# mkln/spamtree

Measured on AMD Instinct MI355X. Metric: Gibbs iterations/sec + achieved HBM GB/s, n=1e6 grid, 1/2/4/8 MI355X, higher is better.
Workload: dtype f64

## Files before the change

include/spamtree_hip.h:

```cpp
#ifndef SPAMTREE_HIP_H
#define SPAMTREE_HIP_H

#include <stdint.h>

#ifdef __cplusplus
extern "C" {
#endif

#define ST_OK 0
#define ST_ERR_CHOL_ROOT 1
#define ST_ERR_CHOL_REF 2
#define ST_ERR_CHOL_LEAF 3
#define ST_ERR_CHOL_SAMPLE_REF 10
#define ST_ERR_CHOL_SAMPLE_LEAF 11
#define ST_ERR_USAGE (-1)
#define ST_ERR_HIP (-2)
#define ST_ERR_TOPOLOGY (-3)
#define ST_ERR_UNSUPPORTED (-4)

#define ST_MAX_Q 6
#define ST_MAX_ANCESTORS 24

typedef struct st_handle_s *st_handle;

// ... 68 lines not shown
int st_get_block(st_handle h, int slot, int64_t u, double *negRiH, double *Ri);
int st_get_comps(st_handle h, int slot, double *logdetCi_comps, double *loglik_w_comps);

int st_algorithmic_bytes(st_handle h, double *out5, double *flops3);
int st_probe_peaks(int device, int64_t bytes, int reps, double *out3);
int st_probe_math(int32_t fn, const double *x, int64_t n, int32_t device, double *out);
#define ST_N_KERNEL_FAMILIES 8
int st_profile_enable(st_handle h, int enable);
int st_profile_get(st_handle h, double *ms_total, int64_t *launches);
int st_profile_levels(st_handle h, int32_t *n_levels, double *ms_by_level, double *bytes_by_level, int32_t cap);
#define ST_KERNEL_GENERIC_LDS 0
#define ST_KERNEL_GENERIC_SCRATCH 1
#define ST_KERNEL_MFMA 2
#define ST_KERNEL_QUAD 3
#define ST_KERNEL_BIGMFMA 4
#define ST_KERNEL_WIDE 5
#define ST_KERNEL_LCHAIN 6
#define ST_KERNEL_LCHAIN_REF 7
int st_level_info(st_handle h, int32_t *n_levels, int32_t *kernel, int32_t *max_m, int32_t *max_P, int32_t *n_blocks, int32_t cap);
#define ST_ROUTE_NONE 0
#define ST_ROUTE_A_SLOTS 3
int st_route_info(st_handle h, int32_t *n_levels, int32_t *phase_a, int32_t *phase_b, int32_t *phase_p, int32_t cap);
const char *st_route_name(int32_t code);
int st_synchronize(st_handle h);
void *st_stream(st_handle h);

int st_cross_covariance_ag10(const double *coords1, const int64_t *mv1, int64_t n1, const double *coords2, const int64_t *mv2,
                             int64_t n2, const double *ai1, const double *ai2, const double *phi_i, const double *thetamv,
                             const double *Dmat, int32_t q, int32_t device, double *out);
int st_summary_reset(st_handle h);
int st_summary_accumulate(st_handle h, uint64_t seed, uint32_t iter);
int st_summary_get(st_handle h, double *w_mean, double *yhat_mean, int64_t *n_accumulated);
int st_summary_reserve(st_handle h, int64_t keep);
int st_summary_quantile(st_handle h, double q, double *w_q, double *yhat_q);

int st_points_set(st_handle h, int64_t n_new, const double *coords, const int64_t *mv, const int64_t *anchor, const double *X);
int st_points_predict(st_handle h, int mode, const double *z, uint64_t seed, uint32_t iter, double *w_new, double *cond_mean,
                      double *cond_var, double *yhat_new);
int st_points_info(st_handle h, int32_t *route, int64_t *n_groups, double *alg_bytes, double *flops);
const char *st_points_route_name(int32_t code);

int st_points_accumulate(st_handle h, uint64_t seed, uint32_t iter, double *w_new, double *cond_mean, double *cond_var, double *yhat_new);
int st_points_summary_reset(st_handle h);
int st_points_summary_reserve(st_handle h, int64_t keep);
int st_points_summary_get(st_handle h, double *mean, double *var, double *w_mean, double *yhat_mean, int64_t *n_accumulated);
int st_points_summary_quantile(st_handle h, double q, double *w_q, double *yhat_q);
// ... 29 lines not shown
```

spamtree_amd/_lib.py:

```python
import ctypes as C
import os

HERE = os.path.dirname(os.path.abspath(__file__))
LIB_PATH = os.environ.get("SPAMTREE_LIB") or os.path.join(HERE, "libspamtree_hip.so")

c_dp = C.POINTER(C.c_double)
c_ip = C.POINTER(C.c_int64)


class StProblem(C.Structure):
    _fields_ = [("n_all", C.c_int64), ("d", C.c_int32), ("q", C.c_int32), ("p", C.c_int32), ("n_groups", C.c_int32),
                ("n_blocks", C.c_int64), ("y", c_dp), ("X", c_dp), ("coords", c_dp), ("mv_id", c_ip),
                ("res_is_ref", c_ip), ("block_names", c_ip), ("block_groups", c_ip), ("indexing_ptr", c_ip),
                ("indexing_idx", c_ip), ("parents_ptr", c_ip), ("parents_idx", c_ip), ("children_ptr", c_ip),
                ("children_idx", c_ip)]


class StOptions(C.Structure):
    _fields_ = [("device", C.c_int32), ("reference_quirks", C.c_int32), ("rank", C.c_int32), ("world", C.c_int32),
                ("force_generic", C.c_int32), ("reserved", C.c_int32)]


H = C.c_void_p
SIGNATURES = {
# ... 14 lines not shown
    "st_sample_w_loglik": (C.c_int, [H, c_dp, C.c_uint64, C.c_uint32, C.c_int, c_dp]),
    "st_sample_w_loglik_begin": (C.c_int, [H, c_dp, C.c_uint64, C.c_uint32, C.c_int]),
    "st_sample_w_loglik_end": (C.c_int, [H, c_dp]),
    "st_predict": (C.c_int, [H, C.c_int]),
    "st_beta_stats": (C.c_int, [H, c_dp]),
    "st_tausq_stats": (C.c_int, [H, c_dp, c_ip]),
    "st_xtx": (C.c_int, [H, c_dp]),
    "st_yhat": (C.c_int, [H, c_dp, C.c_uint64, C.c_uint32, c_dp]),
    "st_block_dims": (C.c_int, [H, C.c_int64, c_ip, c_ip, C.POINTER(C.c_int32), C.POINTER(C.c_int32)]),
    "st_get_block": (C.c_int, [H, C.c_int, C.c_int64, c_dp, c_dp]),
    "st_get_comps": (C.c_int, [H, C.c_int, c_dp, c_dp]),
    "st_algorithmic_bytes": (C.c_int, [H, c_dp, c_dp]),
    "st_factor_ahead_enable": (C.c_int, [H, C.c_int]),
    "st_probe_peaks": (C.c_int, [C.c_int, C.c_int64, C.c_int, c_dp]),
    "st_probe_math": (C.c_int, [C.c_int32, c_dp, C.c_int64, C.c_int32, c_dp]),
    "st_profile_enable": (C.c_int, [H, C.c_int]),
    "st_profile_get": (C.c_int, [H, c_dp, c_ip]),
    "st_profile_levels": (C.c_int, [H, C.POINTER(C.c_int32), c_dp, c_dp, C.c_int32]),
    "st_level_info": (C.c_int, [H, C.POINTER(C.c_int32), C.POINTER(C.c_int32), C.POINTER(C.c_int32), C.POINTER(C.c_int32),
                                C.POINTER(C.c_int32), C.c_int32]),
    "st_route_info": (C.c_int, [H, C.POINTER(C.c_int32), C.POINTER(C.c_int32), C.POINTER(C.c_int32), C.POINTER(C.c_int32),
                                C.c_int32]),
    "st_route_name": (C.c_char_p, [C.c_int32]),
    "st_synchronize": (C.c_int, [H]),
    "st_stream": (C.c_void_p, [H]),
    "st_set_stream": (C.c_int, [H, C.c_void_p]),
    "st_shard_plan": (C.c_int, [C.POINTER(StProblem), C.c_int32, c_ip, C.POINTER(C.c_int32)]),
    "st_shard_plan_opt": (C.c_int, [C.POINTER(StProblem), C.POINTER(StOptions), C.c_int32, c_ip, C.POINTER(C.c_int32)]),
    "st_shard_info": (C.c_int, [H, C.POINTER(C.c_int32), C.POINTER(C.c_int32), C.POINTER(C.c_int32), c_ip, c_ip]),
    "st_factor_local": (C.c_int, [H, C.c_int, c_dp, C.c_int]),
    "st_factor_enqueue": (C.c_int, [H, C.c_int, c_dp, C.c_int]),
    "st_factor_finish": (C.c_int, [H, c_dp]),
    "st_factor_is_async": (C.c_int, [H]),
    "st_loglik_local": (C.c_int, [H, C.c_int]),
    "st_mg_pack_comps": (C.c_int, [H, C.c_int, C.POINTER(C.c_void_p), c_ip]),
    "st_mg_finish": (C.c_int, [H, c_dp]),
    "st_sample_w_local": (C.c_int, [H, c_dp, C.c_uint64, C.c_uint32]),
    "st_mg_top_region": (C.c_int, [H, C.POINTER(C.c_void_p), c_ip]),
    "st_sample_w_top": (C.c_int, [H]),
    "st_mg_pack_w": (C.c_int, [H, C.POINTER(C.c_void_p), c_ip]),
    "st_mg_unpack_w": (C.c_int, [H]),
    "st_mg_gather_w_pack": (C.c_int, [H, C.POINTER(C.c_void_p), C.POINTER(C.c_void_p), c_ip]),
    "st_mg_gather_w_unpack": (C.c_int, [H]),
    "st_cross_covariance_ag10": (C.c_int, [c_dp, c_ip, C.c_int64, c_dp, c_ip, C.c_int64, c_dp, c_dp, c_dp, c_dp, c_dp, C.c_int32,
                                           C.c_int32, c_dp]),
    "st_summary_reset": (C.c_int, [H]),
# ... 70 lines not shown
```

spamtree_amd/csrc/factor_quad.hpp:

```cpp
#pragma once

struct Quad {
  int g0, nu;
  int Jc, Pc;
};

struct QuadArgs {
  const Blk *blks;
  const int *anc_idx;
  const Grp *grps;
  const Quad *quads;
  int nquad;
  const double *cx, *cy;
  const int *mv;
  const double *w;
  double *panels;
  double *logdet_c, *loglik_c;
  int *errflag;
  const long long *gdesc;
  int gd_stride;
  int ldS;
  int wave_chol;
  int predict;
  const double *z;
  double *w_out;
  int mode;
  double *vscr;
  int vtiles;
};

enum { QM_FULL = 0, QM_VONLY = 1, QM_TFROMV = 2 };
__host__ __device__ constexpr int quad_vtiles(int nkx) { return 2 + 2 * ((4 * nkx + 31) / 32); }

#define RFL(x) __builtin_amdgcn_readfirstlane(x)

constexpr int QUAD_LEAF_KH = 5;
__host__ __device__ constexpr int quad_lds_stride(int nkx) {
  int s = 4 * nkx + 24 > 186 ? 4 * nkx + 24 : 186;
  while ((s & 1) || ((s >> 1) & 1) == 0) ++s;
  return s;
}

#ifdef ST_DEFS_FACTOR_QUAD
__device__ __forceinline__ void dma_row(const double *src, double *dst, int Kb, int lane, bool two) {
  if (2 * lane < Kb) __builtin_amdgcn_global_load_lds((q_glb_void *)(src + 2 * lane), (q_lds_void *)dst, 16, 0, 0);
  if (two) {
    if (128 + 2 * lane < Kb) __builtin_amdgcn_global_load_lds((q_glb_void *)(src + 128 + 2 * lane), (q_lds_void *)(dst + 128), 16, 0, 0);
  }
}

template <int NU, int NKX, int NKT, bool ISREF, bool WCH = true>
__global__ __launch_bounds__(128 * NU, 2) void k_factor_quad(QuadArgs A, CovPar cp) {
  constexpr int NTQ = 128 * NU, NW = 2 * NU;
  static_assert(NU >= 2, "s_g overlays two rows of s_e2");
// ... 16 lines not shown
  __shared__ double s_sx[PMAX], s_sy[PMAX], s_wpa[PMAX];
  __shared__ int s_smv[PMAX];
  __shared__ double s_exp2[64];
  __shared__ double s_cvr[QMAX * QMAX], s_cva[QMAX * QMAX], s_cva2[QMAX * QMAX], s_cvp[QMAX];
  __shared__ int s_rlen[PMAX];
  __shared__ long long s_rsrc[PMAX];
  double (*s_g)[32] = s_e2;
  double (*s_gp)[32] = s_hv;

  const int tid = threadIdx.x, lane = tid & 63, l15 = lane & 15, l4 = lane >> 4, ttid = tid & 127;
  const int wid = RFL(tid >> 6), u = wid >> 1, jt = (wid & 1) ^ ((wid >> 2) & 1);
  constexpr int ldS = quad_lds_stride(NKX);
  double *arena = lds;
  double *zrow = arena + (size_t)NU * 16 * ldS;
  double *xch = zrow + ldS;

  STAMP_DECL
  int qidx = blockIdx.x;
  {
    const int per = A.nquad >> 3;
    if (qidx < per * 8) qidx = (qidx & 7) * per + (qidx >> 3);
  }
  const Quad Q = A.quads[qidx];
  const int Jc = Q.Jc, Pc = Q.Pc, nu = Q.nu;

  long long *gdl = (long long *)arena;
  const int gds = A.gd_stride;
  for (int e = tid; e < nu * gds; e += NTQ) {
    const int uu = e / gds, i = e - uu * gds;
    gdl[e] = A.gdesc[(size_t)(Q.g0 + uu) * gds + i];
  }
  for (int k = tid; k < ldS; k += NTQ) zrow[k] = 0.0;
  if (tid < 64) s_exp2[tid] = EXP2_64[tid];
  if (cp.q > 1 && tid >= 64 && tid < 64 + QMAX * QMAX) {
    const int e = tid - 64;
    s_cvr[e] = cp.rate[e]; s_cva[e] = cp.amp[e]; s_cva2[e] = cp.amp2[e];
    if (e < QMAX) s_cvp[e] = cp.phi[e];
  }
  __syncthreads();
  if (tid < NU) {
    int M = 0, P = 0, blk0 = 0, nblk = 0, isref = 0, J = 0, pm = 0;
    long long row0 = 0, prow = 0, ppan = 0;
    if (tid < nu) {
      const long long *g = gdl + (size_t)tid * gds;
      row0 = g[0];
      M = (int)(g[2] & 0xffffffffLL); P = (int)(g[2] >> 32);
// ... 85 lines not shown
    for (int rr = 0; rr < RP; ++rr) {
      const int cc = c0 + min(wid + NW * rr, sr - 1);
      lv[rr] = s_rlen[cc]; sv[rr] = s_rsrc[cc];
    }
#pragma unroll
    for (int rr = 0; rr < RP; ++rr) {
      const int row = wid + NW * rr;
      const int len = RFL(lv[rr]);
      rlen_nx[rr] = len;
      if (row < sr) dma_row(A.panels + sv[rr], buf + (size_t)row * ldS, len, lane, len > 128);
    }
  };
  auto priv_rows = [&](int sp) { return sp == 0 ? p_sr0 : (pmu > 16 ? pmu - p_sr0 : 0); };
  auto priv_issue = [&](int sp, int stride) {
    const int r0 = sp == 0 ? 0 : p_sr0, sr = priv_rows(sp);
    const double *src = A.panels + s_ppan[u] + (size_t)r0 * p_Kb;
    double *buf = arena + (size_t)u * stride * ldS;
#pragma unroll
    for (int rr = 0; rr < 8; ++rr) {
      const int row = jt + 2 * rr;
      if (row < sr) dma_row(src + (size_t)row * p_Kb, buf + (size_t)row * ldS, p_Kb, lane, true);
    }
  };
  if constexpr (ISREF) { if (nit > 0) issue(0, arena); }
  else { if (pmmax > 0) priv_issue(0, 16); }

  double kx[NKX];
  if (QM != QM_TFROMV) {
    const int jc = jt * 16 + l15;
    const bool cok = jc < Mu;
    const double mx = s_colx[u][jc], my = s_coly[u][jc];
    const int mvj = s_colmv[u][jc];
    double *kb = (ISREF ? arena + (size_t)32 * ldS : xch) + (size_t)wid * (KH * 64) + lane;
#pragma unroll
    for (int hpass = 0; hpass < NPASS; ++hpass) {
      const int st0 = hpass * KH;
      if (4 * st0 < Pu) {
        if (cp.q == 1) {
          const double s2 = cp.ai1[0], nphi = -cp.tmv[0];
#pragma unroll 1
          for (int i = 0; i < KH; ++i) {
            const int k = 4 * (st0 + i) + l4;
            double ax = s_sx[min(k, PMAX - 1)], ay = s_sy[min(k, PMAX - 1)];
            if constexpr (!ISREF) {
              if (k >= Pc) { ax = s_px[u][(k - Pc) & 31]; ay = s_py[u][(k - Pc) & 31]; }
            }
            const double dx = ax - mx, dy = ay - my;
            const double v = s2 * cov_exp_tab(nphi * cov_sqrt(fma(dx, dx, dy * dy)), s_exp2);
            kb[i * 64] = (cok && k < Pu) ? v : 0.0;
          }
        } else {
          const int qn = cp.q;
#pragma unroll 1
          for (int i = 0; i < KH; ++i) {
            const int k = 4 * (st0 + i) + l4;
            const double *pxs = &s_sx[min(k, PMAX - 1)], *pys = &s_sy[min(k, PMAX - 1)];
            const int *pvs = &s_smv[min(k, PMAX - 1)];
            if constexpr (!ISREF) {
              if (k >= Pc) { pxs = &s_px[u][(k - Pc) & 31]; pys = &s_py[u][(k - Pc) & 31]; pvs = &s_pmv[u][(k - Pc) & 31]; }
            }
            const int av = *pvs;
            const double dx = *pxs - mx, dy = *pys - my;
            const double hd = cov_sqrt(dx * dx + dy * dy);
            const int ij = av * qn + mvj;
            double v = s_cva[ij] * cov_exp_tab(-s_cvr[ij] * hd, s_exp2);
            v = fma(s_cva2[ij], cov_exp_tab(-s_cvp[av] * hd, s_exp2), v);
            kb[i * 64] = (cok && k < Pu) ? v : 0.0;
          }
        }
#pragma unroll
        for (int i = 0; i < KH; ++i)
          if (st0 + i < NKX) kx[st0 + i] = kb[i * 64];
      } else {
#pragma unroll
        for (int i = 0; i < KH; ++i)
          if (st0 + i < NKX) kx[st0 + i] = 0.0;
      }
    }
  }
  STAMP(1);
  d4 tacc[NKT];
#pragma unroll
  for (int n = 0; n < NKT; ++n) tacc[n] = (d4){0.0, 0.0, 0.0, 0.0};
  d4 rown = (d4){0.0, 0.0, 0.0, 0.0}, rcross = rown;
  double dacc = 0.0;
  double hacc = 0.0;
// ... 472 lines not shown
```

spamtree_amd/csrc/spamtree_hip.hip:

```cpp

#include "st_device.hpp"
#include "factor_generic.hpp"
#include "factor_mfma.hpp"
#include "chol_blocked.hpp"
#include "factor_quad.hpp"
#include "factor_big.hpp"
#include "factor_wide.hpp"
#include "factor_lchain.hpp"
#include "sample_kernels.hpp"
#include "misc_kernels.hpp"
#include "predict_points.hpp"
#include "simulate_kernels.hpp"

static thread_local std::string g_create_error;
struct st_handle_s;
static void points_free(st_handle_s *h);

template <typename T>
struct DevBuf {
  T *p = nullptr;
  size_t n = 0;
  hipError_t alloc(size_t count) {
    n = count;
    if (count == 0) { p = nullptr; return hipSuccess; }
// ... 51 lines not shown
static const char *const k_route_names[R_COUNT] = {
  "",
  "k_marginal_invchol_wave", "k_marginal_invchol",
  "k_factor<false, MODE_FACTOR>", "k_factor<true, MODE_FACTOR>", "k_factor<false, MODE_PREDICT>", "k_factor<true, MODE_PREDICT>",
  "k_factor_quad<4, 32, 8, true, true>", "k_factor_quad<4, 32, 8, true, false>", "k_factor_quad<4, 32, 8, false, true>",
  "k_factor_quad<4, 38, 10, true, true>", "k_factor_quad<4, 38, 10, true, false>", "k_factor_quad<4, 38, 10, false, true>",
  "k_factor_quad<4, 44, 11, true, true>", "k_factor_quad<4, 44, 11, true, false>", "k_factor_quad<4, 44, 11, false, true>",
  "k_factor_quad<4, 50, 13, true, true>", "k_factor_quad<4, 50, 13, true, false>", "k_factor_quad<4, 50, 13, false, true>",
  "k_factor_mfma", "k_factor_lchain<96>", "k_factor_lchain<136>", "k_factor_ref_finish", "k_lchain_scalars", "k_factor_wide<WG_JT>",
  "k_factor_bigmfma<3, 5, 34>", "k_factor_bigmfma<4, 5, 34>", "k_factor_bigmfma<5, 3, 24>",
  "k_gram", "k_gram_direct", "k_gram_big",
  "k_sample_mfma", "k_sample_leaf_seg<4>", "k_sample_leaf_seg<6>", "k_sample_leaf", "k_sample_wave", "k_sample_lean<true>",
  "k_sample_lean<false>", "k_sample<true, false>", "k_sample_leaf_wide", "k_sample<true, true>", "k_sample<false>",
};

struct Switches {
  int wide = 1, split_gram = 1, sample_wave = 1;
  bool lchain = true, lchain_ref = true, gram_big = true, gram_direct = true, sample_lean = true, sample_lat = true,
       leaf_seg = true, leaf_wide = true, async_top = true;
  int lchain_ref_min = 1;
  int factor_gen = 3;
  int quad_units = 0;
  int quad_min = -1;
};

static Switches read_switches() {
  auto level = [](const char *name) {
    const char *e = getenv(name);
    return (e && e[0] == '0') ? 0 : ((e && e[0] == '2') ? 2 : 1);
  };
  Switches s;
  s.wide = level("SPAMTREE_WIDE"); s.split_gram = level("SPAMTREE_SPLIT_GRAM"); s.sample_wave = level("SPAMTREE_SAMPLE_WAVE");
  s.lchain = level("SPAMTREE_LCHAIN"); s.lchain_ref = level("SPAMTREE_LCHAIN_REF"); s.gram_big = level("SPAMTREE_GRAM_BIG");
  s.gram_direct = level("SPAMTREE_GRAM_DIRECT"); s.sample_lean = level("SPAMTREE_SAMPLE_LEAN"); s.sample_lat = level("SPAMTREE_SAMPLE_LAT");
  s.leaf_seg = level("SPAMTREE_LEAF_SEG"); s.leaf_wide = level("SPAMTREE_LEAF_WIDE"); s.async_top = level("SPAMTREE_ASYNC_TOP");
  const char *e;
  if ((e = getenv("SPAMTREE_LCHAIN_REF_MIN"))) s.lchain_ref_min = atoi(e);
  if ((e = getenv("SPAMTREE_FACTOR_KERNEL")) && e[0] == '1') s.factor_gen = 1;
  if ((e = getenv("SPAMTREE_QUAD_UNITS"))) s.quad_units = atoi(e);
  if ((e = getenv("SPAMTREE_QUAD_MIN"))) s.quad_min = std::max(atoi(e), 0);
  return s;
}

struct st_handle_s {
  std::string err;
  int device = 0;
  hipStream_t stream = nullptr;
  int quirks = 1, force_generic = 0;
  Switches sw;
  long long n_all = 0, n_blocks = 0;
  int q = 1, p = 1, d = 2, n_groups = 0, n_actual_groups = 0;
  long long n_obs = 0;
  size_t lds_limit = 65536;
  int sm_count = 256;

  std::vector<long long> dev2model, model2dev;
  std::vector<int> blk_model2dev;
  std::vector<Blk> blks;
  std::vector<int> anc_idx, dch_idx, lvl_list, pred_list, all_obs_list;
  std::vector<Grp> grps;
  DevBuf<Grp> d_grps;
  std::vector<Quad> quads;
  DevBuf<Quad> d_quads;
// ... 41 lines not shown
  bool ext_stream = false;
  DevBuf<double> d_sum_w, d_sum_yhat;
  long long n_summary = 0;
  DevBuf<double> d_draws_w, d_draws_yhat;
  long long draws_cap = 0, n_draws = 0;
  int gram_direct_level = -1;
  bool stats_valid = false;
  bool host_stats_valid = false;
  std::vector<double> host_stats;
  double *pin = nullptr;
  double *pin_up = nullptr;
  int pin_up_slot = 0, pin_up_len = 0;
  hipEvent_t ev_up[2] = {nullptr, nullptr};
  bool factor_open = false; int factor_open_slot = 0;
  std::vector<double> top_theta_open;
  hipEvent_t ev_factor = nullptr;
  std::vector<char> s0_valid;
  bool gram_valid = false;
  bool cache_gram = true;
  bool defer_leaf = false;
  bool leaf_pending[2] = {false, false};
  CovPar leaf_cp[2];
  DevBuf<double> d_vleaf;
  bool limited = false;
  std::vector<int> twin_list;
  DevBuf<int> d_twin;
  int twin_maxM = 1;
  ncclComm_t comm = nullptr;
  std::vector<LevelInfo> levels;
  std::vector<int> route_a, route_b;
  int route_p = R_NONE;
  LevelInfo pred_info;
  int pred_grp_first = 0, pred_grp_count = 0, pred_quad_first = 0, pred_quad_count = 0, pred_nkx = 0;
  size_t pred_lds = 0;
  std::vector<double> xtx;
  std::vector<long long> n_obs_q;
  struct PointSet *pts = nullptr;
  DevBuf<double> d_simz, d_sime, d_simw, d_simy;
  DevBuf<int> d_rowblk;
  int sim_cap = 0;
  std::vector<SimLevel> sim_levels;

  DevBuf<double> d_cx, d_cy, d_y, d_X, d_w, d_xb, d_z, d_B, d_panels[2], d_acc, d_logdet[2], d_loglik[2], d_scalars, d_partial,
      d_stats, d_scratch, d_tmp_n, d_tsq;
  DevBuf<int> d_mv, d_anc, d_dch, d_lvl, d_pred, d_allobs, d_err;
  DevBuf<unsigned char> d_obs;
// ... 88 lines not shown
}
static size_t scratch_factor_doubles(int maxP, int maxM, int maxMa) {
  return (size_t)2 * maxP * maxM + (size_t)maxMa * maxM + (size_t)2 * maxM * maxM;
}
static size_t lds_sample_sq_bytes(int maxM) { return ((size_t)maxM * ((maxM + 7) | 1) + maxM + 16) * 8; }
static size_t lds_sample_bytes(int maxP, int maxM, int maxLd, bool big) {
  size_t dbl = (size_t)(maxP + maxM) + 4 * (size_t)maxM + (size_t)MAXJ * maxM;
  if (!big) dbl += (size_t)maxM * maxLd + (size_t)maxM * maxM;
  return dbl * 8 + 64;
}
static size_t lds_loglik_bytes(int maxP, int maxM) { return ((size_t)maxP + 2 * (size_t)maxM) * 8 + 64; }

extern "C" const char *st_last_error(st_handle h) { return h ? h->err.c_str() : g_create_error.c_str(); }
extern "C" void st_set_create_error(const char *msg) { g_create_error = msg ? msg : ""; }

extern "C" int st_destroy(st_handle h) {
  if (!h) return ST_OK;
  (void)hipSetDevice(h->device);
  h->d_cx.free(); h->d_cy.free(); h->d_y.free(); h->d_X.free(); h->d_w.free(); h->d_xb.free(); h->d_z.free(); h->d_B.free();
  h->d_panels[0].free(); h->d_panels[1].free(); h->d_acc.free();
  for (int s = 0; s < 2; ++s) { h->d_logdet[s].free(); h->d_loglik[s].free(); }
  h->d_scalars.free(); h->d_partial.free(); h->d_stats.free(); h->d_scratch.free(); h->d_tmp_n.free(); h->d_tsq.free();
  h->d_mv.free(); h->d_anc.free(); h->d_dch.free(); h->d_lvl.free(); h->d_pred.free(); h->d_allobs.free(); h->d_err.free();
  h->d_twin.free(); h->d_wgrps.free(); h->d_lcslabs.free(); h->d_lcrow.free(); h->d_rfvoff.free(); h->d_vscr.free(); h->d_vleaf.free(); h->d_s0.free(); h->d_s0off.free(); h->d_obs.free(); h->d_dev2model.free(); h->d_partner.free(); h->d_blks.free(); h->d_grps.free(); h->d_quads.free(); h->d_gdesc.free();
  h->d_ownobs.free(); h->d_owngrp.free(); h->d_ownslow.free(); h->d_rowmask.free(); h->d_blkmask.free(); h->d_comm.free(); h->d_gather.free(); h->d_gidx.free(); h->d_gerr.free(); h->d_err2.free(); h->d_toplist.free();
  if (h->ev_top) (void)hipEventDestroy(h->ev_top);
  if (h->ev_main) (void)hipEventDestroy(h->ev_main);
  if (h->ev_stats) (void)hipEventDestroy(h->ev_stats);
  if (h->stream2) (void)hipStreamDestroy(h->stream2); h->d_sum_w.free(); h->d_sum_yhat.free(); h->d_draws_w.free(); h->d_draws_yhat.free();
  prof_harvest(h);
  for (auto e : h->ev_free) (void)hipEventDestroy(e);
  if (h->comm) (void)ncclCommDestroy(h->comm);
  if (h->pin) (void)hipHostFree(h->pin);
  if (h->pin_up) (void)hipHostFree(h->pin_up);
  for (int i = 0; i < 2; ++i) if (h->ev_up[i]) (void)hipEventDestroy(h->ev_up[i]);
  if (h->ev_factor) (void)hipEventDestroy(h->ev_factor);
  points_free(h);
  h->d_simz.free(); h->d_sime.free(); h->d_simw.free(); h->d_simy.free(); h->d_rowblk.free();
  if (h->stream && !h->ext_stream) (void)hipStreamDestroy(h->stream);
  delete h;
  return ST_OK;
}

static int create_impl(const st_problem *pb, const st_options *opt, st_handle *out, bool plan_only, int64_t *owner_out, int32_t *cut_out);

extern "C" int st_create(const st_problem *pb, const st_options *opt, st_handle *out) {
  return create_impl(pb, opt, out, false, nullptr, nullptr);
// ... 852 lines not shown
      if (hipFuncGetAttributes(&fa, fr) == hipSuccess) stat = std::max(stat, (size_t)fa.sharedSizeBytes);
      const void *ft = (const void *)k_factor_quad<4, 50, 13, true, false>;
      if (hipFuncGetAttributes(&fa, ft) == hipSuccess) stat = std::max(stat, (size_t)fa.sharedSizeBytes);
    }
    for (auto &L : h->levels) {
      if (L.q_nkx == 0) continue;
      if (L.lds_quad + stat > 160 * 1024) L.q_nkx = 0;
    }
    if (h->pred_nkx && h->pred_lds + stat > 160 * 1024) h->pred_nkx = 0;
#define QATTR(NU_, NKX_, NKT_)                                                                                                       \
  (void)hipFuncSetAttribute((const void *)k_factor_quad<NU_, NKX_, NKT_, true, true>, hipFuncAttributeMaxDynamicSharedMemorySize, 160 * 1024 - (int)stat); \
  (void)hipFuncSetAttribute((const void *)k_factor_quad<NU_, NKX_, NKT_, true, false>, hipFuncAttributeMaxDynamicSharedMemorySize, 160 * 1024 - (int)stat); \
  (void)hipFuncSetAttribute((const void *)k_factor_quad<NU_, NKX_, NKT_, false, true>, hipFuncAttributeMaxDynamicSharedMemorySize, 160 * 1024 - (int)stat)
    QATTR(4, 50, 13); QATTR(4, 44, 11); QATTR(4, 38, 10); QATTR(4, 32, 8);
#undef QATTR
    size_t vl = 0;
    for (auto &L : h->levels) {
      L.vl_off = -1;
      if (!h->defer_leaf || h->world > 1 || h->limited || h->sw.factor_gen != 3 || !L.fast || L.isref || L.q_nkx == 0 || L.qown_n == 0) continue;
      L.vl_off = (long long)vl;
      vl += (size_t)L.qown_n * quad_vtiles(L.q_nkx) * (2 * h->quad_nu) * 256;
    }
    if (vl) CCHK(h->d_vleaf.alloc(vl));
  }
  {
    h->g_top = 0;
    bool all_fast = !h->limited && !h->force_generic;
    for (int g = 0; g < n_actual; ++g) all_fast = all_fast && h->levels[g].fast;
    if (all_fast) {
      while (h->g_top < n_actual && !(h->sw.factor_gen == 3 && h->levels[h->g_top].q_nkx > 0)) ++h->g_top;
      if (h->g_top >= n_actual) h->g_top = 0;
    }
    h->async_top = h->g_top > 0 && h->sw.async_top;
    std::vector<int> tl;
    for (int b : h->own_obs_list) if (h->blks[b].level < h->g_top) tl.push_back(b);
    h->n_toplist = (int)tl.size();
    if (tl.empty()) tl.push_back(0);
    CCHK(h->d_toplist.upload(tl));
    CCHK(h->d_err2.alloc(2));
    if (h->async_top) {
      CCHK(hipStreamCreateWithFlags(&h->stream2, hipStreamNonBlocking));
      CCHK(hipEventCreateWithFlags(&h->ev_top, hipEventDisableTiming));
      CCHK(hipEventCreateWithFlags(&h->ev_main, hipEventDisableTiming));
      CCHK(hipEventCreateWithFlags(&h->ev_stats, hipEventDisableTiming));
    }
  }
// ... 218 lines not shown
      hipLaunchKernelGGL(k_marginal_invchol, dim3(std::min(M.nlist, 8 * h->sm_count)), dim3(NT), lds, st, M, cp);
    }
  }
  for (int g = g_lo; g < g_hi; ++g) {
    const LevelInfo &L = h->levels[g];
    if ((L.fast ? L.gown_n : L.own_n) == 0) continue;
    FactorArgs A;
    std::memset(&A, 0, sizeof(A));
    A.blks = h->d_blks.p; A.anc_idx = h->d_anc.p; A.list = h->d_lvl.p + L.first + L.own_lo; A.nlist = L.own_n;
    A.cx = h->d_cx.p; A.cy = h->d_cy.p; A.mv = h->d_mv.p; A.w_in = h->d_w.p; A.w_out = nullptr; A.z = nullptr;
    A.panels = h->d_panels[phys].p; A.logdet_c = h->d_logdet[phys].p; A.loglik_c = h->d_loglik[phys].p;
    A.errflag = errflag; A.maxP = L.maxP; A.maxM = L.maxM; A.maxMa = L.maxMa; A.SR = L.big_factor ? 4 : 8;
    {
      ProfScope ps(h, 0, g, 1, st);
      if (L.fast && h->sw.factor_gen == 3 && L.q_nkx > 0) {
        QuadArgs F;
        std::memset(&F, 0, sizeof(F));
        F.blks = h->d_blks.p; F.anc_idx = h->d_anc.p; F.grps = h->d_grps.p + L.grp_first;
        F.quads = h->d_quads.p + L.quad_first + L.qown_lo; F.nquad = L.qown_n;
        F.cx = h->d_cx.p; F.cy = h->d_cy.p; F.mv = h->d_mv.p; F.w = h->d_w.p; F.panels = h->d_panels[phys].p;
        F.logdet_c = h->d_logdet[phys].p; F.loglik_c = h->d_loglik[phys].p; F.errflag = errflag; F.ldS = L.q_ldS;
        F.gdesc = h->d_gdesc.p + (size_t)L.grp_first * h->gd_stride; F.gd_stride = h->gd_stride;
        F.wave_chol = L.maxM <= 27 ? 1 : 0;
#define QLAUNCH(NU_, NKX_, NKT_, R_)     \
  do {                                                                                                                         \
    if (L.isref && F.wave_chol) { route(g, R_); hipLaunchKernelGGL((k_factor_quad<NU_, NKX_, NKT_, true, true>), dim3(L.qown_n), dim3(128 * NU_), L.lds_quad, st, F, cp); } \
    else if (L.isref) { route(g, R_ + 1); hipLaunchKernelGGL((k_factor_quad<NU_, NKX_, NKT_, true, false>), dim3(L.qown_n), dim3(128 * NU_), L.lds_quad, st, F, cp); } \
    else {                                                                                                                     \
      if (vonly && L.vl_off >= 0) { F.mode = QM_VONLY; F.vscr = h->d_vleaf.p + L.vl_off; F.vtiles = quad_vtiles(NKX_); *deferred = true; } \
      route(g, R_ + 2); hipLaunchKernelGGL((k_factor_quad<NU_, NKX_, NKT_, false, true>), dim3(L.qown_n), dim3(128 * NU_), L.lds_quad, st, F, cp); } \
  } while (0)
        if (L.q_nkx == 32) QLAUNCH(4, 32, 8, R_QUAD32_REF_WCH); else if (L.q_nkx == 38) QLAUNCH(4, 38, 10, R_QUAD38_REF_WCH);
        else if (L.q_nkx == 44) QLAUNCH(4, 44, 11, R_QUAD44_REF_WCH); else QLAUNCH(4, 50, 13, R_QUAD50_REF_WCH);
#undef QLAUNCH
      } else if (L.fast) {
        FastArgs F;
        std::memset(&F, 0, sizeof(F));
        F.blks = h->d_blks.p; F.anc_idx = h->d_anc.p; F.grps = h->d_grps.p + L.grp_first + L.gown_lo; F.ngrp = L.gown_n;
        F.cx = h->d_cx.p; F.cy = h->d_cy.p; F.mv = h->d_mv.p; F.w = h->d_w.p; F.panels = h->d_panels[phys].p;
        F.logdet_c = h->d_logdet[phys].p; F.loglik_c = h->d_loglik[phys].p; F.errflag = errflag;
        F.Pm4 = L.Pm4; F.ldKV = L.ldKV; F.ldS = L.ldS; F.SRm = L.SRm; F.stage_dbl = L.stage_dbl;
        F.gdesc = h->d_gdesc.p + (size_t)(L.grp_first + L.gown_lo) * h->gd_stride; F.gd_stride = h->gd_stride;
        route(g, R_FACTOR_MFMA);
        hipLaunchKernelGGL(k_factor_mfma, dim3(L.gown_n), dim3(NT), L.lds_fast, st, F, cp);
      } else if (L.bigmfma && h->sw.factor_gen == 3 && L.lchain) {
        LcArgs C;
        std::memset(&C, 0, sizeof(C));
        C.blks = h->d_blks.p; C.anc_idx = h->d_anc.p; C.slabs = h->d_lcslabs.p + L.lc_first; C.nslab = L.lc_count;
        C.cx = h->d_cx.p; C.cy = h->d_cy.p; C.mv = h->d_mv.p; C.w_in = h->d_w.p; C.panels = h->d_panels[phys].p;
        C.rowtmp = h->d_lcrow.p; C.n_rows = h->n_all; C.errflag = errflag;
        C.errcode = L.lchain_ref ? 2 : 3;
        C.vscr = L.lchain_ref ? h->d_vscr.p : nullptr;
        if (L.lchain == 96) { route(g, R_LCHAIN96); hipLaunchKernelGGL((k_factor_lchain<96>), dim3(L.lc_count), dim3(LC_NT), lc_dyn_doubles(96) * 8, st, C, cp); }
        else { route(g, R_LCHAIN136); hipLaunchKernelGGL((k_factor_lchain<136>), dim3(L.lc_count), dim3(LC_NT), lc_dyn_doubles(136) * 8, st, C, cp); }
        if (L.lchain_ref) {
          A.vscr = h->d_vscr.p; A.voff = h->d_rfvoff.p + L.rf_first; A.hvrow = h->d_lcrow.p;
          route(g, R_REF_FINISH);
// ... 838 lines not shown
    if (bytes_by_level) bytes_by_level[g] = g < ng ? h->levels[g].alg_bytes_A : h->levels[g - ng].alg_bytes_B + h->levels[g - ng].alg_bytes_msg;
    h->prof_level_ms[g] = 0.0; h->prof_level_n[g] = 0;
  }
  return ST_OK;
}

extern "C" int st_level_info(st_handle h, int32_t *n_levels, int32_t *kernel, int32_t *max_m, int32_t *max_P, int32_t *n_blocks, int32_t cap) {
  if (!h || !n_levels) return ST_ERR_USAGE;
  *n_levels = h->n_actual_groups;
  for (int g = 0; g < h->n_actual_groups && g < cap; ++g) {
    const LevelInfo &L = h->levels[g];
    int k = L.big_factor ? ST_KERNEL_GENERIC_SCRATCH : ST_KERNEL_GENERIC_LDS;
    if (L.fast && h->sw.factor_gen == 3 && L.q_nkx > 0) k = ST_KERNEL_QUAD;
    else if (L.fast) k = ST_KERNEL_MFMA;
    else if (L.bigmfma && h->sw.factor_gen == 3) k = L.lchain ? (L.lchain_ref ? ST_KERNEL_LCHAIN_REF : ST_KERNEL_LCHAIN) : (L.wide_count > 0 ? ST_KERNEL_WIDE : ST_KERNEL_BIGMFMA);
    if (kernel) kernel[g] = k;
    if (max_m) max_m[g] = L.maxM;
    if (max_P) max_P[g] = L.maxP;
    if (n_blocks) n_blocks[g] = L.count;
  }
  return ST_OK;
}

extern "C" int st_route_info(st_handle h, int32_t *n_levels, int32_t *phase_a, int32_t *phase_b, int32_t *phase_p, int32_t cap) {
  if (!h || !n_levels) return ST_ERR_USAGE;
  *n_levels = h->n_actual_groups;
  for (int g = 0; g < h->n_actual_groups && g < cap; ++g) {
    for (int i = 0; i < ST_ROUTE_A_SLOTS && phase_a; ++i) phase_a[ST_ROUTE_A_SLOTS * g + i] = h->route_a[(size_t)ST_ROUTE_A_SLOTS * g + i];
    for (int i = 0; i < 2 && phase_b; ++i) phase_b[2 * g + i] = h->route_b[2 * (size_t)g + i];
  }
  if (phase_p) *phase_p = h->route_p;
  return ST_OK;
}
extern "C" const char *st_route_name(int32_t code) { return (code >= 0 && code < R_COUNT) ? k_route_names[code] : nullptr; }

extern "C" int st_cross_covariance_ag10(const double *coords1, const int64_t *mv1, int64_t n1, const double *coords2, const int64_t *mv2,
                                        int64_t n2, const double *ai1, const double *ai2, const double *phi_i, const double *thetamv,
                                        const double *Dmat, int32_t q, int32_t device, double *out) {
  if (!coords1 || !coords2 || !mv1 || !mv2 || !out || !Dmat || q < 2 || q > QMAX) {
    g_create_error = q < 2 ? "Invalid Dmat for multivariate data" : "st_cross_covariance_ag10: bad argument";
    return ST_ERR_USAGE;
  }
  if (n1 < 0 || n2 < 0) { g_create_error = "st_cross_covariance_ag10: negative extent"; return ST_ERR_USAGE; }
  if (n1 == 0 || n2 == 0) return ST_OK;
  if (hipSetDevice(device) != hipSuccess) { g_create_error = "no usable HIP device"; return ST_ERR_HIP; }
  CovPar cp;
// ... 550 lines not shown
```

spamtree_amd/fit.py:

```python
from __future__ import annotations

import ctypes as C

import numpy as np

from . import _lib
from .model import SpamTreeError, _dp, _f64, _i64, _ip, _lists_to_csr


def _problem(y, X, coords, mv_id, res_is_ref, parents, children, block_names, block_groups, indexing):
    y = _f64(np.asarray(y).reshape(-1))
    X = np.asfortranarray(np.asarray(X, dtype=np.float64))
    coords = np.asfortranarray(np.asarray(coords, dtype=np.float64))
    mv_id = _i64(mv_id)
    ip, ii = indexing if isinstance(indexing, tuple) else _lists_to_csr(indexing)
    pp, pi = parents if isinstance(parents, tuple) else _lists_to_csr(parents)
    cp, ci = children if isinstance(children, tuple) else _lists_to_csr(children)
    keep = [y, X, coords, mv_id, _i64(res_is_ref), _i64(block_names), _i64(block_groups), _i64(ip), _i64(ii), _i64(pp),
            _i64(pi), _i64(cp), _i64(ci)]
    n, p = X.shape
    q = int(np.unique(mv_id).size)
    pb = _lib.StProblem(n, coords.shape[1], q, p, int(keep[4].size), int(keep[5].size), _dp(y), _dp(X), _dp(coords),
                        _ip(mv_id), *[_ip(a) for a in keep[4:]])
    return pb, keep, n, p, q
# ... 81 lines not shown

    def profile(self, enable):
        self.lib.st_profile_enable(self.h, 2 if enable == 2 else int(bool(enable)))

    def profile_get(self):
        ms, n = np.zeros(8), np.zeros(8, dtype=np.int64)
        self.lib.st_profile_get(self.h, _dp(ms), _ip(n))
        names = ["factor", "sample", "loglik", "reduce", "stats", "rng", "predict", "comm"]
        return {k: (float(ms[i]), int(n[i])) for i, k in enumerate(names)}

    def profile_levels(self):
        nl = C.c_int32(); ms = np.zeros(64); by = np.zeros(64)
        self.lib.st_profile_levels(self.h, C.byref(nl), _dp(ms), _dp(by), 64)
        return ms[: nl.value].copy(), by[: nl.value].copy()

    def profile_levels_all(self):
        nl = C.c_int32(); ms = np.zeros(128); by = np.zeros(128)
        self.lib.st_profile_levels(self.h, C.byref(nl), _dp(ms), _dp(by), 128)
        k = nl.value
        return ms[:k].copy(), by[:k].copy(), ms[k: 2 * k].copy(), by[k: 2 * k].copy()

    def factor_ahead_levels(self):
        return int(self.lib.st_factor_ahead_levels(self.h))

    def synchronize(self):
        self.lib.st_synchronize(self.h)

    def shard_info(self):
        r, w, c = C.c_int32(), C.c_int32(), C.c_int32()
        ob, orow = C.c_int64(), C.c_int64()
        self.lib.st_shard_info(self.h, C.byref(r), C.byref(w), C.byref(c), C.byref(ob), C.byref(orow))
        return dict(rank=r.value, world=w.value, cut_level=c.value, owned_blocks=ob.value, owned_rows=orow.value)

    def close(self):
        if self.c:
            self.lib.stm_destroy(self.c)
            self.c = None

    def __del__(self):
        try:
            self.close()
        except Exception:
            pass


def _points_inputs(new_points, p, q, new_quantiles):
# ... 104 lines not shown
```

spamtree_amd/model.py:

```python
from __future__ import annotations

import ctypes as C

import numpy as np

from . import _lib


def _f64(a):
    return np.ascontiguousarray(a, dtype=np.float64)


def _i64(a):
    return np.ascontiguousarray(a, dtype=np.int64)


def _dp(a):
    return a.ctypes.data_as(_lib.c_dp)


def _ip(a):
    return a.ctypes.data_as(_lib.c_ip)


# ... 256 lines not shown
    def level_info(self):
        nl = C.c_int32()
        arr = [np.zeros(64, dtype=np.int32) for _ in range(4)]
        ptr = [a.ctypes.data_as(C.POINTER(C.c_int32)) for a in arr]
        self._check(self.lib.st_level_info(self.h, C.byref(nl), ptr[0], ptr[1], ptr[2], ptr[3], 64))
        return [dict(kernel=self.KERNEL_NAMES[arr[0][g]], max_m=int(arr[1][g]), max_P=int(arr[2][g]), n_blocks=int(arr[3][g]))
                for g in range(nl.value)]

    def route_info(self):
        nl = C.c_int32()
        cap = 64
        a = np.zeros(3 * cap, dtype=np.int32)
        b = np.zeros(2 * cap, dtype=np.int32)
        p = C.c_int32()
        ip = C.POINTER(C.c_int32)
        self._check(self.lib.st_route_info(self.h, C.byref(nl), a.ctypes.data_as(ip), b.ctypes.data_as(ip), C.byref(p), cap))

        def name(code):
            return self.lib.st_route_name(int(code)).decode() if code else None
        levels = [dict(A=[name(c) for c in a[3 * g:3 * g + 3] if c], gram=name(b[2 * g]), sweep=name(b[2 * g + 1]))
                  for g in range(min(nl.value, cap))]
        return dict(levels=levels, predict=name(p.value))

    def synchronize(self):
        self._check(self.lib.st_synchronize(self.h))

    def set_points(self, coords, mv, anchor, X=None):
        coords = np.asfortranarray(np.asarray(coords, dtype=np.float64).reshape(-1, 2))
        n = coords.shape[0]
        mv = _i64(np.asarray(mv).reshape(-1))
        anchor = _i64(np.asarray(anchor).reshape(-1))
        if mv.size != n or anchor.size != n:
            raise ValueError("coords, mv and anchor must describe the same points")
        Xf = None
        if X is not None:
            Xf = np.asfortranarray(np.asarray(X, dtype=np.float64).reshape(n, self.p))
        self._check(self.lib.st_points_set(self.h, n, _dp(coords), _ip(mv), _ip(anchor), _dp(Xf) if Xf is not None else None))
        self.n_points = n
        self.points_have_X = Xf is not None

    def predict_points(self, mode=0, z=None, seed=0, it=0):
        n = self.n_points
        out = {k: np.zeros(n) for k in ("w", "mean", "var")}
        out["yhat"] = np.zeros(n) if self.points_have_X else None
        zz = _f64(np.asarray(z).reshape(-1)) if z is not None else None
        if zz is not None and zz.size != n:
# ... 19 lines not shown
```

Before: 239.3.

## Cache pairwise distances across factorizations in quad factor kernel

Adds a per-level device buffer that stores the pairwise distances computed in the quad factor kernel on the first factorization. Later factorizations load these distances with nontemporal loads instead of recomputing sqrt from the coordinates. This trades sqrt and LDS coordinate work for extra HBM traffic and up to 16 GiB of memory. It also adds a waitcnt before the DMA issue and a query API. Coordinates are fixed across iterations, so reusing the distances is legitimate.

```diff
diff --git a/include/spamtree_hip.h b/include/spamtree_hip.h
--- a/include/spamtree_hip.h
+++ b/include/spamtree_hip.h
@@ -114,6 +114,7 @@
 #define ST_ROUTE_A_SLOTS 3
 int st_route_info(st_handle h, int32_t *n_levels, int32_t *phase_a, int32_t *phase_b, int32_t *phase_p, int32_t cap);
 const char *st_route_name(int32_t code);
+int st_dist_cache_info(st_handle h, int64_t *bytes, int32_t *levels_cached, int32_t *levels_quad);
 int st_synchronize(st_handle h);
 void *st_stream(st_handle h);
 
diff --git a/profiles/quad_isa_waits.py b/profiles/quad_isa_waits.py
--- /dev/null
+++ b/profiles/quad_isa_waits.py
@@ -0,0 +1,16 @@
+#!/usr/bin/env python3
+import re
+import subprocess
+import sys
+
+txt = open(sys.argv[1]).read()
+for m in re.finditer(r"^(_Z13k_factor_quad\w+):.*?^\.Lfunc_end\d+:", txt, re.S | re.M):
+    name = subprocess.run(["c++filt", m.group(1)], capture_output=True, text=True).stdout.strip()
+    lines = m.group(0).splitlines()
+    d = next(i for i, l in enumerate(lines) if "global_load_lds" in l)
+    w = next(i for i in range(d + 1, len(lines)) if "vmcnt(" in lines[i])
+    span = lines[d:w]
+    cnt = lambda s: sum(s in l for l in span)
+    print(f"{name}: first DMA at line {d}, next vmcnt wait {w - d} lines on: {lines[w].strip()} | in between: "
+          f"{cnt('v_rsq_f64')} v_rsq_f64, {cnt('v_ldexp_f64')} v_ldexp_f64, {cnt('global_load_dwordx2')} global loads, "
+          f"{cnt('global_store_dwordx2')} global stores")
diff --git a/spamtree_amd/_lib.py b/spamtree_amd/_lib.py
--- a/spamtree_amd/_lib.py
+++ b/spamtree_amd/_lib.py
@@ -60,6 +60,7 @@
     "st_route_info": (C.c_int, [H, C.POINTER(C.c_int32), C.POINTER(C.c_int32), C.POINTER(C.c_int32), C.POINTER(C.c_int32),
                                 C.c_int32]),
     "st_route_name": (C.c_char_p, [C.c_int32]),
+    "st_dist_cache_info": (C.c_int, [H, c_ip, C.POINTER(C.c_int32), C.POINTER(C.c_int32)]),
     "st_synchronize": (C.c_int, [H]),
     "st_stream": (C.c_void_p, [H]),
     "st_set_stream": (C.c_int, [H, C.c_void_p]),
diff --git a/spamtree_amd/csrc/factor_quad.hpp b/spamtree_amd/csrc/factor_quad.hpp
--- a/spamtree_amd/csrc/factor_quad.hpp
+++ b/spamtree_amd/csrc/factor_quad.hpp
@@ -27,9 +27,13 @@
   int mode;
   double *vscr;
   int vtiles;
+  int dmode;
+  double *dist;
 };
 
 enum { QM_FULL = 0, QM_VONLY = 1, QM_TFROMV = 2 };
+enum { QD_OFF = 0, QD_FILL = 1, QD_LOAD = 2 };
+__host__ __device__ constexpr size_t quad_dist_doubles(int nkx) { return (size_t)nkx * 8 * 64; }
 __host__ __device__ constexpr int quad_vtiles(int nkx) { return 2 + 2 * ((4 * nkx + 31) / 32); }
 
 #define RFL(x) __builtin_amdgcn_readfirstlane(x)
@@ -92,6 +96,13 @@
     if (qidx < per * 8) qidx = (qidx & 7) * per + (qidx >> 3);
   }
   const Quad Q = A.quads[qidx];
+  const int DM = RFL(A.dmode);
+  double kx[NKX];
+  const double *dq = A.dist + ((size_t)qidx * NKX * NW + wid) * 64;
+  if (DM == QD_LOAD) {
+#pragma unroll
+    for (int st = 0; st < NKX; ++st) kx[st] = __builtin_nontemporal_load(dq + (size_t)st * (NW * 64) + lane);
+  }
   const int Jc = Q.Jc, Pc = Q.Pc, nu = Q.nu;
 
   long long *gdl = (long long *)arena;
@@ -223,31 +234,43 @@
       if (row < sr) dma_row(src + (size_t)row * p_Kb, buf + (size_t)row * ldS, p_Kb, lane, true);
     }
   };
+  __builtin_amdgcn_s_waitcnt(0x0F70);
   if constexpr (ISREF) { if (nit > 0) issue(0, arena); }
   else { if (pmmax > 0) priv_issue(0, 16); }
 
-  double kx[NKX];
   if (QM != QM_TFROMV) {
     const int jc = jt * 16 + l15;
     const bool cok = jc < Mu;
     const double mx = s_colx[u][jc], my = s_coly[u][jc];
     const int mvj = s_colmv[u][jc];
+    double *dqs = const_cast<double *>(dq) + lane;
     double *kb = (ISREF ? arena + (size_t)32 * ldS : xch) + (size_t)wid * (KH * 64) + lane;
 #pragma unroll
     for (int hpass = 0; hpass < NPASS; ++hpass) {
       const int st0 = hpass * KH;
       if (4 * st0 < Pu) {
+        if (DM == QD_LOAD) {
+#pragma unroll
+          for (int i = 0; i < KH; ++i)
+            if (st0 + i < NKX) kb[i * 64] = kx[st0 + i];
+        }
         if (cp.q == 1) {
           const double s2 = cp.ai1[0], nphi = -cp.tmv[0];
 #pragma unroll 1
           for (int i = 0; i < KH; ++i) {
             const int k = 4 * (st0 + i) + l4;
-            double ax = s_sx[min(k, PMAX - 1)], ay = s_sy[min(k, PMAX - 1)];
-            if constexpr (!ISREF) {
-              if (k >= Pc) { ax = s_px[u][(k - Pc) & 31]; ay = s_py[u][(k - Pc) & 31]; }
+            double hd;
+            if (DM == QD_LOAD) hd = kb[i * 64];
+            else {
+              double ax = s_sx[min(k, PMAX - 1)], ay = s_sy[min(k, PMAX - 1)];
+              if constexpr (!ISREF) {
+                if (k >= Pc) { ax = s_px[u][(k - Pc) & 31]; ay = s_py[u][(k - Pc) & 31]; }
+              }
+              const double dx = ax - mx, dy = ay - my;
+              hd = cov_sqrt(fma(dx, dx, dy * dy));
+              if (DM == QD_FILL && st0 + i < NKX) __builtin_nontemporal_store(hd, dqs + (size_t)(st0 + i) * (NW * 64));
             }
-            const double dx = ax - mx, dy = ay - my;
-            const double v = s2 * cov_exp_tab(nphi * cov_sqrt(fma(dx, dx, dy * dy)), s_exp2);
+            const double v = s2 * cov_exp_tab(nphi * hd, s_exp2);
             kb[i * 64] = (cok && k < Pu) ? v : 0.0;
           }
         } else {
@@ -261,8 +284,13 @@
               if (k >= Pc) { pxs = &s_px[u][(k - Pc) & 31]; pys = &s_py[u][(k - Pc) & 31]; pvs = &s_pmv[u][(k - Pc) & 31]; }
             }
             const int av = *pvs;
-            const double dx = *pxs - mx, dy = *pys - my;
-            const double hd = cov_sqrt(dx * dx + dy * dy);
+            double hd;
+            if (DM == QD_LOAD) hd = kb[i * 64];
+            else {
+              const double dx = *pxs - mx, dy = *pys - my;
+              hd = cov_sqrt(dx * dx + dy * dy);
+              if (DM == QD_FILL && st0 + i < NKX) __builtin_nontemporal_store(hd, dqs + (size_t)(st0 + i) * (NW * 64));
+            }
             const int ij = av * qn + mvj;
             double v = s_cva[ij] * cov_exp_tab(-s_cvr[ij] * hd, s_exp2);
             v = fma(s_cva2[ij], cov_exp_tab(-s_cvp[av] * hd, s_exp2), v);
diff --git a/spamtree_amd/csrc/spamtree_hip.hip b/spamtree_amd/csrc/spamtree_hip.hip
--- a/spamtree_amd/csrc/spamtree_hip.hip
+++ b/spamtree_amd/csrc/spamtree_hip.hip
@@ -97,6 +97,8 @@
   int factor_gen = 3;
   int quad_units = 0;
   int quad_min = -1;
+  bool dist_cache = true;
+  long long dist_cache_max = 16LL << 30;
 };
 
 static Switches read_switches() {
@@ -114,6 +116,8 @@
   if ((e = getenv("SPAMTREE_FACTOR_KERNEL")) && e[0] == '1') s.factor_gen = 1;
   if ((e = getenv("SPAMTREE_QUAD_UNITS"))) s.quad_units = atoi(e);
   if ((e = getenv("SPAMTREE_QUAD_MIN"))) s.quad_min = std::max(atoi(e), 0);
+  s.dist_cache = level("SPAMTREE_DIST_CACHE");
+  if ((e = getenv("SPAMTREE_DIST_CACHE_MAX"))) s.dist_cache_max = std::max(atoll(e), 0LL);
   return s;
 }
 
@@ -201,6 +205,8 @@
   bool leaf_pending[2] = {false, false};
   CovPar leaf_cp[2];
   DevBuf<double> d_vleaf;
+  std::vector<DevBuf<double>> d_dist;
+  std::vector<char> dist_valid;
   bool limited = false;
   std::vector<int> twin_list;
   DevBuf<int> d_twin;
@@ -335,7 +341,7 @@
   for (int s = 0; s < 2; ++s) { h->d_logdet[s].free(); h->d_loglik[s].free(); }
   h->d_scalars.free(); h->d_partial.free(); h->d_stats.free(); h->d_scratch.free(); h->d_tmp_n.free(); h->d_tsq.free();
   h->d_mv.free(); h->d_anc.free(); h->d_dch.free(); h->d_lvl.free(); h->d_pred.free(); h->d_allobs.free(); h->d_err.free();
-  h->d_twin.free(); h->d_wgrps.free(); h->d_lcslabs.free(); h->d_lcrow.free(); h->d_rfvoff.free(); h->d_vscr.free(); h->d_vleaf.free(); h->d_s0.free(); h->d_s0off.free(); h->d_obs.free(); h->d_dev2model.free(); h->d_partner.free(); h->d_blks.free(); h->d_grps.free(); h->d_quads.free(); h->d_gdesc.free();
+  h->d_twin.free(); h->d_wgrps.free(); h->d_lcslabs.free(); h->d_lcrow.free(); h->d_rfvoff.free(); h->d_vscr.free(); h->d_vleaf.free(); for (auto &b : h->d_dist) b.free(); h->d_s0.free(); h->d_s0off.free(); h->d_obs.free(); h->d_dev2model.free(); h->d_partner.free(); h->d_blks.free(); h->d_grps.free(); h->d_quads.free(); h->d_gdesc.free();
   h->d_ownobs.free(); h->d_owngrp.free(); h->d_ownslow.free(); h->d_rowmask.free(); h->d_blkmask.free(); h->d_comm.free(); h->d_gather.free(); h->d_gidx.free(); h->d_gerr.free(); h->d_err2.free(); h->d_toplist.free();
   if (h->ev_top) (void)hipEventDestroy(h->ev_top);
   if (h->ev_main) (void)hipEventDestroy(h->ev_main);
@@ -1234,6 +1240,17 @@
       vl += (size_t)L.qown_n * quad_vtiles(L.q_nkx) * (2 * h->quad_nu) * 256;
     }
     if (vl) CCHK(h->d_vleaf.alloc(vl));
+    h->d_dist.assign(h->levels.size(), DevBuf<double>());
+    h->dist_valid.assign(h->levels.size(), 0);
+    size_t dc_bytes = 0;
+    for (size_t g = 0; g < h->levels.size() && h->sw.dist_cache; ++g) {
+      const LevelInfo &L = h->levels[g];
+      if (h->sw.factor_gen != 3 || !L.fast || L.q_nkx == 0 || L.qown_n == 0) continue;
+      const size_t cnt = (size_t)L.qown_n * quad_dist_doubles(L.q_nkx);
+      if (dc_bytes + cnt * sizeof(double) > (size_t)h->sw.dist_cache_max) continue;
+      if (h->d_dist[g].alloc(cnt) != hipSuccess) { (void)hipGetLastError(); h->d_dist[g].p = nullptr; h->d_dist[g].n = 0; continue; }
+      dc_bytes += cnt * sizeof(double);
+    }
   }
   {
     h->g_top = 0;
@@ -1498,6 +1515,8 @@
         F.logdet_c = h->d_logdet[phys].p; F.loglik_c = h->d_loglik[phys].p; F.errflag = errflag; F.ldS = L.q_ldS;
         F.gdesc = h->d_gdesc.p + (size_t)L.grp_first * h->gd_stride; F.gd_stride = h->gd_stride;
         F.wave_chol = L.maxM <= 27 ? 1 : 0;
+        const bool dc = (size_t)g < h->d_dist.size() && h->d_dist[g].p && st == h->stream;
+        if (dc) { F.dmode = h->dist_valid[g] ? QD_LOAD : QD_FILL; F.dist = h->d_dist[g].p; }
 #define QLAUNCH(NU_, NKX_, NKT_, R_)     \
   do {                                                                                                                         \
     if (L.isref && F.wave_chol) { route(g, R_); hipLaunchKernelGGL((k_factor_quad<NU_, NKX_, NKT_, true, true>), dim3(L.qown_n), dim3(128 * NU_), L.lds_quad, st, F, cp); } \
@@ -1509,6 +1528,7 @@
         if (L.q_nkx == 32) QLAUNCH(4, 32, 8, R_QUAD32_REF_WCH); else if (L.q_nkx == 38) QLAUNCH(4, 38, 10, R_QUAD38_REF_WCH);
         else if (L.q_nkx == 44) QLAUNCH(4, 44, 11, R_QUAD44_REF_WCH); else QLAUNCH(4, 50, 13, R_QUAD50_REF_WCH);
 #undef QLAUNCH
+        if (dc && hipPeekAtLastError() == hipSuccess) h->dist_valid[g] = 1;
       } else if (L.fast) {
         FastArgs F;
         std::memset(&F, 0, sizeof(F));
@@ -2393,6 +2413,20 @@
   return ST_OK;
 }
 
+extern "C" int st_dist_cache_info(st_handle h, int64_t *bytes, int32_t *levels_cached, int32_t *levels_quad) {
+  if (!h) return ST_ERR_USAGE;
+  long long b = 0; int nc = 0, nq = 0;
+  for (int g = 0; g < h->n_actual_groups; ++g) {
+    const LevelInfo &L = h->levels[g];
+    if (L.fast && h->sw.factor_gen == 3 && L.q_nkx > 0 && L.qown_n > 0) ++nq;
+    if ((size_t)g < h->d_dist.size() && h->d_dist[g].p) { ++nc; b += (long long)(h->d_dist[g].n * sizeof(double)); }
+  }
+  if (bytes) *bytes = b;
+  if (levels_cached) *levels_cached = nc;
+  if (levels_quad) *levels_quad = nq;
+  return ST_OK;
+}
+
 extern "C" int st_route_info(st_handle h, int32_t *n_levels, int32_t *phase_a, int32_t *phase_b, int32_t *phase_p, int32_t cap) {
   if (!h || !n_levels) return ST_ERR_USAGE;
   *n_levels = h->n_actual_groups;
diff --git a/spamtree_amd/fit.py b/spamtree_amd/fit.py
--- a/spamtree_amd/fit.py
+++ b/spamtree_amd/fit.py
@@ -127,6 +127,11 @@
 
     def factor_ahead_levels(self):
         return int(self.lib.st_factor_ahead_levels(self.h))
+
+    def dist_cache_info(self):
+        b, nc, nq = C.c_int64(), C.c_int32(), C.c_int32()
+        self.lib.st_dist_cache_info(self.h, C.byref(b), C.byref(nc), C.byref(nq))
+        return dict(bytes=b.value, levels_cached=nc.value, levels_quad=nq.value)
 
     def synchronize(self):
         self.lib.st_synchronize(self.h)
diff --git a/spamtree_amd/model.py b/spamtree_amd/model.py
--- a/spamtree_amd/model.py
+++ b/spamtree_amd/model.py
@@ -302,6 +302,11 @@
                   for g in range(min(nl.value, cap))]
         return dict(levels=levels, predict=name(p.value))
 
+    def dist_cache_info(self):
+        b, nc, nq = C.c_int64(), C.c_int32(), C.c_int32()
+        self._check(self.lib.st_dist_cache_info(self.h, C.byref(b), C.byref(nc), C.byref(nq)))
+        return dict(bytes=b.value, levels_cached=nc.value, levels_quad=nq.value)
+
     def synchronize(self):
         self._check(self.lib.st_synchronize(self.h))
 
```

After: 231.2. 0.966x the previous value.
